# david-zwicker/video-analysis

Measured on AMD Instinct MI355X. Metric: frames/sec (bg-sub+blur+thresh+CCL) 1080p uint8, higher is better.
Workload: dtype u8; 1 GPU; cfg3_1080p_full_chain: 1920x1080 uint8, batch 256/GPU, running-mean bg-sub (f64 state) + sigma=5 Gaussian (q8.8) + threshold 20 + 5x5 dilate/erode + 4-connected labelling + object counts; inputs resident in HBM; engine=bg=1 gauss=mfma-i8(ksize=31) thresh=20 morph=2 ccl=4, video=one clip per rank, overlap=off, world_size=1, backend=single process

## Files before the change

video-analysis_amd/csrc/va_api.hip:

```cpp
#include <dlfcn.h>
#include <stdarg.h>
#include <stdlib.h>

#include <mutex>
#include <vector>
#include <new>

#include "va_common.h"

namespace va {

static thread_local char g_err[512] = "";

void set_error(const char *fmt, ...)
{
    va_list ap;
    va_start(ap, fmt);
    vsnprintf(g_err, sizeof(g_err), fmt, ap);
    va_end(ap);
}
const char *get_error() { return g_err; }

struct ScratchBlock {
    void *ptr;
    size_t bytes;
    hipStream_t st;
};
static std::mutex g_scratch_mu;
static std::vector<ScratchBlock> g_scratch_free;
static size_t g_scratch_cached = 0;
constexpr size_t kScratchCacheCap = 6ull << 30;

static void scratch_release_all_locked()
{
    for (const ScratchBlock &b : g_scratch_free)
        (void)hipFree(b.ptr);
    g_scratch_free.clear();
    g_scratch_cached = 0;
}

struct ScratchLease {
// ... 394 lines not shown
        return rc;
    return launch_gaussian(g, src, dst, nullptr, -1, 0, scratch.ptr, n, as_stream(stream), nullptr);
}

int va_gaussian_u8(const uint8_t *src, uint8_t *dst, int n, int h, int w, int c, double sigma,
                   void *stream)
{
    return va_gaussian_u8_rule(src, dst, n, h, w, c, sigma, VA_TAPS_CV4, stream);
}

int va_gaussian_u8_rule(const uint8_t *src, uint8_t *dst, int n, int h, int w, int c, double sigma,
                        int tap_rule, void *stream)
{
    return gaussian_call("va_gaussian_u8", VA_U8, src, dst, n, h, w, c, sigma, tap_rule, GaussFamily::None,
                         stream);
}

int va_gaussian_u8_generic(const uint8_t *src, uint8_t *dst, int n, int h, int w, int c,
                           double sigma, void *stream)
{
    return gaussian_call("va_gaussian_u8_generic", VA_U8, src, dst, n, h, w, c, sigma, VA_TAPS_CV4,
                         GaussFamily::U8Generic, stream);
}

int va_gaussian_u8_valu(const uint8_t *src, uint8_t *dst, int n, int h, int w, int c, double sigma,
                        void *stream)
{
    return gaussian_call("va_gaussian_u8_valu", VA_U8, src, dst, n, h, w, c, sigma, VA_TAPS_CV4,
                         GaussFamily::U8Dot, stream);
}

int va_test_hook_labelling(int path, int lds_runs)
{
    VA_REQUIRE(path >= 0 && path <= 4 && lds_runs >= 0, "va_test_hook_labelling: bad arguments");
    ccl_test_hook(path, lds_runs);
    return VA_OK;
}

static int g_gauss_u8_valu = 0;
int va_test_hook_gaussian_u8(int force_valu)
{
    g_gauss_u8_valu = force_valu != 0;
    return VA_OK;
}

int va_test_hook_gaussian_f32(int generic_columns)
{
    gauss_f32_test_hook(generic_columns);
    return VA_OK;
}

int va_gaussian_f32(const float *src, float *dst, int n, int h, int w, int c, double sigma,
                    void *stream)
{
    return gaussian_call("va_gaussian_f32", VA_F32, src, dst, n, h, w, c, sigma, VA_TAPS_CV4, GaussFamily::None,
                         stream);
}

int va_bg_update(int mode, int dtype, const void *frames, void *diff_out, void *state,
                 int64_t n_seen, double rate, int n, size_t px, void *stream)
{
    VA_ENTER();
    double *recip = nullptr;
    ScratchLease scratch;
    if (mode == VA_BG_MEAN && dtype == VA_U8 && n > 0) {
        int rc = scratch.acquire(bg_scratch_bytes(n), as_stream(stream));
        if (rc)
// ... 882 lines not shown
    uint32_t *const *bits = p->bits[slot];

    bool have_bits = false;
    if (c.sigma > 0) {
        if (p->gauss.byte_mask() && masks && mask_out && !filtered_out && c.morph_count == 0 && !want_ccl &&
            reinterpret_cast<uintptr_t>(mask_out) % 4 == 0) {
            return launch_gaussian(p->gauss, cur, mask_out, nullptr, c.thresh, c.maxval, p->gscratch, n, st, prof);
        }
        uint32_t *gbits = masks && p->gauss.single_pass() ? bits[0] : nullptr;
        void *dst = filtered_out ? filtered_out : p->blur;
        rc = launch_gaussian(p->gauss, cur, dst, gbits, c.thresh, 0, p->gscratch, n, st, prof);
        if (rc)
            return rc;
        have_bits = gbits != nullptr;
        cur = dst;
    } else if (filtered_out) {
        VA_HIP(hipMemcpyAsync(filtered_out, cur, (size_t)n * p->px * esz, hipMemcpyDeviceToDevice,
                              st));
    }
    if (!masks)
        return VA_OK;

    int b = 0;
    if (!have_bits) {
        rc = launch_pack_bits((const uint8_t *)cur, bits[0], n, c.height, c.width, c.thresh, st);
        if (rc)
            return rc;
        VA_MARK("threshold_pack");
    }
    int32_t *labels = nullptr;
    if (want_ccl) {
        labels = labels_out ? labels_out : p->labels_scratch;
    }
    if (c.morph_count > 0 && morph_fused_supported(c.width, p->se, c.morph_count)) {
        rc = launch_morph_fused(bits[b], bits[b ^ 1], n, c.height, c.width, c.morph_op, p->se,
                                c.morph_count, st);
        if (rc)
            return rc;
        b ^= 1;
        VA_MARK("morph_fused");
    } else {
        for (int i = 0; i < c.morph_count; i++) {
            rc = launch_morph_bits(bits[b], bits[b ^ 1], n, c.height, c.width, c.morph_op[i],
                                   p->se[i], st);
            if (rc)
                return rc;
            b ^= 1;
            VA_MARK(c.morph_op[i] == VA_MORPH_DILATE ? "morph_dilate" : "morph_erode");
        }
    }
    if (mask_out) {
        rc = launch_unpack_bits(bits[b], mask_out, n, c.height, c.width, c.maxval, st);
        if (rc)
            return rc;
        VA_MARK("mask_unpack");
    }
    if (want_ccl) {
        const bool paint = labels_out != nullptr || stats_out != nullptr;
        int32_t *counts = counts_out ? counts_out : p->counts_scratch;
        const char *lo = (const char *)labels, *hi = lo + (size_t)n * p->frame_px * sizeof(int32_t);
        const char *slo = (const char *)stats_out,
                   *shi = slo + (stats_out ? (size_t)n * c.max_labels * VA_STATS_STRIDE * sizeof(int64_t) : 0);
        for (int s = 0; s < 2 && p->overlap; s++)
            if (p->paint_pending[s] &&
                ((lo < p->paint_hi[s] && p->paint_lo[s] < hi) || (slo < p->pstat_hi[s] && p->pstat_lo[s] < shi)))
                VA_HIP(hipStreamWaitEvent(st, p->ev_paint[s], 0));
        if (!defer_paint) {
            rc = launch_ccl(bits[b], labels, counts, n, c.height, c.width, c.connectivity, p->ccl_ws[0],
                            p->ccl_ws_bytes, stats_out, c.max_labels, st, prof, paint);
            if (rc)
                return rc;
        } else {
            CclPaintPlan plan;
            rc = launch_ccl_front(bits[b], labels, counts, n, c.height, c.width, c.connectivity, p->ccl_ws[slot],
                                  p->ccl_ws_bytes, stats_out, c.max_labels, st, prof, &plan);
            if (rc)
                return rc;
            VA_HIP(hipEventRecord(p->ev_front, st));
            VA_HIP(hipStreamWaitEvent(p->side, p->ev_front, 0));
            if (prof)
                prof->mark(nullptr, p->side);
            plan.persistent_grid = p->paint_grid;
            rc = launch_ccl_paint(plan, p->side, prof);
            if (rc)
                return rc;
            VA_HIP(hipEventRecord(p->ev_paint[slot], p->side));
            p->paint_pending[slot] = true;
            p->paint_lo[slot] = lo;
            p->paint_hi[slot] = hi;
            p->pstat_lo[slot] = slo;
            p->pstat_hi[slot] = shi;
            p->slot = slot ^ 1;
        }
    }
#undef VA_MARK
    return VA_OK;
}

int va_pipeline_profile(va_pipeline_t *p, int enable)
{
    VA_ENTER();
    VA_REQUIRE(p, "va_pipeline_profile: NULL pipeline");
    if (!p->prof) {
        p->prof = new (std::nothrow) StageProfiler();
        if (!p->prof) {
            set_error("va_pipeline_profile: out of host memory");
            return VA_ERR_NOMEM;
        }
// ... 154 lines not shown
```

video-analysis_amd/csrc/va_ccl.hip:

```cpp
#include "va_common.h"

namespace va {

namespace {

constexpr int kBlock = 256;
constexpr int kRowsPerBlock = kBlock / kWave;
constexpr bool kNtStores = true;

__device__ __forceinline__ int ld_forest(const int32_t *p)
{
    return __hip_atomic_load(p, __ATOMIC_RELAXED, __HIP_MEMORY_SCOPE_WORKGROUP);
}
__device__ __forceinline__ void st_forest(int32_t *p, int v)
{
    __hip_atomic_store(p, v, __ATOMIC_RELAXED, __HIP_MEMORY_SCOPE_WORKGROUP);
}

__device__ int find_root(int32_t *L, int a)
{
    for (;;) {
        int p = ld_forest(L + a);
        if (p == a)
            return a;
        int gp = ld_forest(L + p);
        if (gp == p)
            return p;
        st_forest(L + a, gp);
        a = gp;
    }
}

__device__ int find_root_ro(const int32_t *L, int a)
// ... 547 lines not shown
        all += p;
    }
    if (threadIdx.x == 0)
        *total = all;
    __syncthreads();
    return before + incl - v;
}

__device__ __forceinline__ void scan_rows(int *rowbase, int h, int *s_part, int *total)
{
    const int per = (h + kFrameThreads - 1) / kFrameThreads;
    const int y0 = min(h, (int)threadIdx.x * per), y1 = min(h, y0 + per);
    int sum = 0;
    for (int y = y0; y < y1; y++)
        sum += rowbase[y];
    int run = block_exclusive_scan(sum, s_part, total);
    for (int y = y0; y < y1; y++) {
        const int n = rowbase[y];
        rowbase[y] = run;
        run += n;
    }
    __syncthreads();
}

#ifdef VA_CCL_STAMPS
__device__ long long g_ccl_stamps[16];
__device__ int g_ccl_xcc[2][16];
#define CCL_ACC(v, t0) do { long long t1_ = __builtin_amdgcn_s_memtime(); v += t1_ - t0; t0 = t1_; } while (0)
#define CCL_STAMP(i) do { if (blockIdx.x == 0 && threadIdx.x == 0) g_ccl_stamps[i] = __builtin_amdgcn_s_memtime(); } while (0)
#else
#define CCL_STAMP(i) do { } while (0)
#define CCL_ACC(v, t0) do { } while (0)
#endif
template <bool CONN8, int NCH, int RPW>
__global__ void __launch_bounds__(kFrameThreads)
ccl_frame_kernel(const uint32_t *__restrict__ bits, int32_t *__restrict__ labels,
                 int32_t *__restrict__ counts, int h, int w, int w32, FrameLayout lay, int direct,
                 int32_t *__restrict__ table, int table_stride, int32_t *__restrict__ rowbase_g,
                 int32_t *__restrict__ mode)
{
    __shared__ __attribute__((aligned(16))) int s_mem[kFrameLdsWords];
    __shared__ int s_part[kFrameWaves];
    __shared__ int s_total;

    const int f = blockIdx.x, tid = threadIdx.x, wv = tid >> 6, lane = tid & (kWave - 1);
#ifdef VA_CCL_STAMPS
    if (tid == 0 && f < 16)
        g_ccl_xcc[0][f] = __builtin_amdgcn_s_getreg((3 << 11) | 20) & 15;
#endif
    const uint32_t *fbits = bits + (size_t)f * h * w32;
    int32_t *L = labels + (size_t)f * h * w;
    int *stage = s_mem + wv * lay.stage_words + kStagePad;
    const int rs = lay.row_stride;
    const bool spans_direct = NCH == 1 && direct;
    if (!spans_direct)
        for (int i = lane; i < lay.stage_words; i += kWave)
            stage[i - kStagePad] = 0;
    int *queue = s_mem + lay.queue_off + wv * 2 * kQueue;
    int *rowbase = s_mem + lay.rowbase_off;
    int *parent = s_mem + lay.parent_off;
    constexpr int kRowsPerIter = kFrameWaves * RPW;
    const int sweeps = (h + kRowsPerIter - 1) / kRowsPerIter;

    typedef int v4i __attribute__((ext_vector_type(4)));
    struct RowRegs {
        v4i v[RPW + 1];
    };
    const int nld = (w32 + kWave - 1) / kWave;
    auto issue_rows = [&](int y0, RowRegs &rr) {
        const int c0 = min(lane, w32 - 1), c1 = min(lane + kWave, w32 - 1);
        const int c2 = min(lane + 2 * kWave, w32 - 1), c3 = min(lane + 3 * kWave, w32 - 1);
#pragma unroll
        for (int j = 0; j <= RPW; j++) {
            const uint32_t *src = fbits + (size_t)min(max(y0 - 1 + j, 0), h - 1) * w32;
            rr.v[j].x = (int)src[c0];
            if (nld > 1)
                rr.v[j].y = (int)src[c1];
            if (nld > 2) {
                rr.v[j].z = (int)src[c2];
                rr.v[j].w = (int)src[c3];
            }
        }
    };
// ... 976 lines not shown
        if (n++ == 0) {
            x = px;
            y = py;
        }
    }
};

__global__ void longest_contour_start_kernel(const uint32_t *__restrict__ bits,
                                             const unsigned long long *__restrict__ best_idx, int h, int w,
                                             int w32, int32_t *__restrict__ p1)
{
    const int f = blockIdx.x;
    if (threadIdx.x != 0)
        return;
    const unsigned long long key = best_idx[f];
    FirstEmit e;
    if (key != 0) {
        const int idx = (int)key - 1;
        BitImage im{bits + (size_t)f * h * w32, h, w, w32};
        trace_outer_border(im, idx % w, idx / w, e);
    }
    p1[2 * f] = e.x;
    p1[2 * f + 1] = e.y;
}

inline bool aligned(const void *p, size_t a) { return (reinterpret_cast<uintptr_t>(p) % a) == 0; }

}

static int g_ccl_path = 0;
static int g_ccl_lds_runs = 0;
static int g_ccl_sparse = 0;
static int g_ccl_no_direct = 0;
void ccl_test_hook(int path, int lds_runs)
{
    g_ccl_sparse = path == 3;
    g_ccl_no_direct = path == 4;
    g_ccl_path = path == 4 ? 2 : path == 3 ? 0 : path;
    g_ccl_lds_runs = lds_runs;
}

static int frame_rows_per_wave(int h, int w32)
{
    if ((long long)h * w32 > kMaxFrameWords || w32 > 128)
        return 0;
    for (int rpw = 8; rpw >= 4; rpw >>= 1)
        if (span_chunks(w32, rpw) <= 2 &&
            frame_layout(h, w32, rpw).lds_runs >= (rpw == 8 ? kWantLdsRuns : kMinLdsRuns))
            return rpw;
    return span_chunks(w32, 8) <= 2 && frame_layout(h, w32, 8).lds_runs >= kMinLdsRuns ? 8 : 0;
}

bool ccl_frame_kernel_used(int n, int h, int w)
{
    if (g_ccl_path == 1)
        return false;
    const int rpw = frame_rows_per_wave(h, words_per_row(w));
    if (rpw == 0)
        return false;
    if (g_ccl_path != 2) {
        const double wf = (double)h * words_per_row(w) / 64800.0, fill = (double)min(n, 256) / 256.0;
        const double t_frame = wf * (rpw == 8 ? 0.04 + 0.066 * fill : 0.075) + 0.01;
        const double t_chip = 0.277 * wf * n / 256.0 + 0.03;
        if (t_frame >= t_chip)
            return false;
    }
    return true;
}

static inline size_t up256(size_t v) { return (v + 255) & ~(size_t)255; }
size_t ccl_rows_workspace_bytes(int n, int h)
{
    return 2 * up256((size_t)n * h * sizeof(int32_t)) + up256((size_t)n * kFrameLdsWords * sizeof(int32_t)) +
           up256((size_t)n * sizeof(int32_t));
}

size_t ccl_workspace_bytes(int n, int h, int w)
{
    size_t bits = (size_t)n * h * words_per_row(w) * sizeof(uint32_t);
    auto up = [](size_t v) { return (v + 255) & ~(size_t)255; };
    return up(bits) + ccl_rows_workspace_bytes(n, h);
}

int launch_ccl_front(const uint32_t *bits, int32_t *labels, int32_t *counts, int n, int h, int w,
                     int connectivity, void *workspace, size_t ws_bytes, int64_t *stats, int max_labels,
                     hipStream_t st, StageProfiler *prof, CclPaintPlan *plan)
{
    const bool paint = plan != nullptr;
    if (plan)
        plan->n = 0;
#define VA_MARK(nm)      \
    do {                 \
        if (prof)        \
            prof->mark(nm, st); \
    } while (0)
    VA_REQUIRE(connectivity == 4 || connectivity == 8, "label: connectivity must be 4 or 8 (got %d)",
               connectivity);
    VA_REQUIRE(bits && labels && workspace, "label: NULL argument");
    VA_REQUIRE((size_t)h * (size_t)w < kMaxFramePixels,
               "label: frames of %dx%d exceed the supported 2^29 pixels (32-bit buffer descriptors "
               "address h*w*4 bytes of labels)", w, h);
    if (n == 0 || h == 0 || w == 0)
        return VA_OK;
    const int w32 = words_per_row(w);
    const size_t total_rows = (size_t)n * h;
    auto up = [](size_t v) { return (v + 255) & ~(size_t)255; };
    VA_REQUIRE(ws_bytes >= ccl_rows_workspace_bytes(n, h), "label: workspace too small");
    int32_t *row_cnt = (int32_t *)workspace;
    int32_t *row_off = (int32_t *)((char *)workspace + up(total_rows * sizeof(int32_t)));
    int32_t *run_table = (int32_t *)((char *)workspace + 2 * up(total_rows * sizeof(int32_t)));
    int32_t *frame_mode = (int32_t *)((char *)run_table + up((size_t)n * kFrameLdsWords * sizeof(int32_t)));
    bool table_mode = false;
    int table_stride = 0;

    const dim3 sgrid_all((unsigned)cdiv(h, kSparseRowsPerBlock), (unsigned)min(n, 4096));
    FrameList all{nullptr, nullptr, n};
    auto chip_wide = [&](const dim3 &sgrid, const FrameList &fl, int nscan, bool init) -> int {
        if (init) {
            ccl_init_kernel<<<sgrid, kBlock, 0, st>>>(bits, labels, h, w, w32, fl);
            VA_LAUNCH_CHECK("ccl_init_kernel");
            VA_MARK("ccl_init");
        }
        if (connectivity == 8)
            ccl_link_kernel<true><<<sgrid, kBlock, 0, st>>>(bits, labels, h, w, w32, fl);
        else
            ccl_link_kernel<false><<<sgrid, kBlock, 0, st>>>(bits, labels, h, w, w32, fl);
        VA_LAUNCH_CHECK("ccl_link_kernel");
        VA_MARK("ccl_link");
        ccl_flatten_kernel<<<sgrid, kBlock, 0, st>>>(bits, labels, row_cnt, h, w, w32, fl);
        VA_LAUNCH_CHECK("ccl_flatten_kernel");
        VA_MARK("ccl_flatten");
        ccl_rowscan_kernel<<<nscan, kBlock, 0, st>>>(row_cnt, row_off, counts, h, fl);
        VA_LAUNCH_CHECK("ccl_rowscan_kernel");
        VA_MARK("ccl_rowscan");
        ccl_rank_kernel<<<sgrid, kBlock, 0, st>>>(bits, labels, row_off, h, w, w32, fl);
        VA_LAUNCH_CHECK("ccl_rank_kernel");
        VA_MARK("ccl_rank");
        return VA_OK;
    };
    if (ccl_frame_kernel_used(n, h, w)) {
        const int rpw = frame_rows_per_wave(h, w32);
        FrameLayout lay = frame_layout(h, w32, rpw);
        if (g_ccl_lds_runs > 0)
            lay.lds_runs = min(lay.lds_runs, g_ccl_lds_runs);
        const int nch = span_chunks(w32, rpw);
        const int direct = nch == 1 && (w32 % 4 == 0) && aligned(bits, 16) && !g_ccl_no_direct;
        table_mode = paint && !g_ccl_sparse;
        table_stride = lay.lds_runs;
#define VA_FRAME_LAUNCH(C8, NCH, RPW)                                                                       \
    ccl_frame_kernel<C8, NCH, RPW><<<n, kFrameThreads, 0, st>>>(bits, labels, counts, h, w, w32, lay, direct,  \
                                                                 table_mode ? run_table : nullptr, lay.lds_runs, \
                                                                 row_off, frame_mode)
#define VA_FRAME_CASE(NCH, RPW)                 \
    if (nch == NCH && rpw == RPW) {             \
        if (connectivity == 8)                  \
            VA_FRAME_LAUNCH(true, NCH, RPW);    \
        else                                    \
            VA_FRAME_LAUNCH(false, NCH, RPW);   \
    }
        VA_FRAME_CASE(1, 8) VA_FRAME_CASE(2, 8) VA_FRAME_CASE(1, 4) VA_FRAME_CASE(2, 4)
#undef VA_FRAME_CASE
#undef VA_FRAME_LAUNCH
        VA_LAUNCH_CHECK("ccl_frame_kernel");
        VA_MARK("ccl_frame");
    } else {
        int rc = chip_wide(sgrid_all, all, n, true);
        if (rc)
            return rc;
    }
    if (!paint)
        return VA_OK;
    plan->bits = bits;
    plan->labels = labels;
    plan->n = n;
    plan->h = h;
    plan->w = w;
    plan->stats = stats;
    plan->max_labels = max_labels;
    plan->run_table = table_mode ? run_table : nullptr;
    plan->table_stride = table_stride;
    plan->row_off = row_off;
    plan->frame_mode = frame_mode;
    plan->xcd_frames = table_mode ? cdiv(h, kRowsPerBlock) : 0;
    plan->persistent_grid = 0;
#undef VA_MARK
    return VA_OK;
}

int launch_ccl_paint(const CclPaintPlan &pl, hipStream_t st, StageProfiler *prof)
{
#define VA_MARK(nm)      \
// ... 9 lines not shown
    const int grid = cdiv((long long)total_rows, kRowsPerBlock);
    const int vblocks = pl.xcd_frames ? 8 * pl.xcd_frames * cdiv(n, 8) : grid;
    const int pgrid = pl.persistent_grid > 0 ? min(vblocks, pl.persistent_grid) : vblocks;
    const bool wide = w32 > kWave && w32 <= 2 * kWave && vec && (w & 3) == 0 && (h & (kRowsPerBlock - 1)) == 0;
#define VA_PAINT_LAUNCH(ST, WORDS, STATSP, ML)                                                                      \
    ccl_paint_kernel<ST, WORDS><<<pgrid, kBlock, 0, st>>>(pl.bits, pl.labels, h, w, w32, total_rows, STATSP, ML, vec, \
                                                        pl.run_table, pl.table_stride, pl.row_off, pl.frame_mode,    \
                                                        pl.xcd_frames, vblocks)
    if (pl.stats && pl.max_labels > 0) {
        size_t entries = (size_t)n * pl.max_labels;
        stats_init_kernel<<<cdiv((long long)entries * VA_STATS_STRIDE, kBlock), kBlock, 0, st>>>(
            pl.stats, entries, h, w);
        VA_LAUNCH_CHECK("stats_init_kernel");
        VA_MARK("stats_init");
        if (wide)
            VA_PAINT_LAUNCH(true, 2 * kWave, pl.stats, pl.max_labels);
        else
            VA_PAINT_LAUNCH(true, kWave, pl.stats, pl.max_labels);
    } else {
        if (wide)
            VA_PAINT_LAUNCH(false, 2 * kWave, nullptr, 0);
        else
            VA_PAINT_LAUNCH(false, kWave, nullptr, 0);
    }
#undef VA_PAINT_LAUNCH
    VA_LAUNCH_CHECK("ccl_paint_kernel");
    VA_MARK("ccl_paint");
#undef VA_MARK
    return VA_OK;
}

int launch_ccl(const uint32_t *bits, int32_t *labels, int32_t *counts, int n, int h, int w,
               int connectivity, void *workspace, size_t ws_bytes, int64_t *stats, int max_labels,
               hipStream_t st, StageProfiler *prof, bool paint)
{
    CclPaintPlan plan;
    int rc = launch_ccl_front(bits, labels, counts, n, h, w, connectivity, workspace, ws_bytes, stats, max_labels,
                              st, prof, paint ? &plan : nullptr);
    if (rc || !paint)
        return rc;
    return launch_ccl_paint(plan, st, prof);
}

int launch_stats_from_labels(const int32_t *labels, int n, int h, int w, int max_labels,
                             int64_t *stats, hipStream_t st)
{
    VA_REQUIRE(labels && stats && max_labels > 0, "moments: NULL argument / max_labels <= 0");
    if (n == 0 || h == 0 || w == 0)
        return VA_OK;
    size_t entries = (size_t)n * max_labels;
    stats_init_kernel<<<cdiv((long long)entries * VA_STATS_STRIDE, kBlock), kBlock, 0, st>>>(
        stats, entries, h, w);
    VA_LAUNCH_CHECK("stats_init_kernel");
    const int w32 = words_per_row(w);
    size_t total_words = (size_t)n * h * w32;
    stats_from_labels_kernel<<<cdiv((long long)total_words, kBlock), kBlock, 0, st>>>(
        labels, h, w, w32, total_words, stats, max_labels);
    VA_LAUNCH_CHECK("stats_from_labels_kernel");
    return VA_OK;
}

int launch_largest_region(const int32_t *labels, const int32_t *counts, const int64_t *stats,
                          int n, int h, int w, int max_labels, int32_t *largest,
                          int64_t *largest_area, uint8_t *mask_out, hipStream_t st)
{
    VA_REQUIRE(counts && stats && largest && max_labels > 0, "largest_region: NULL argument");
    if (n == 0)
        return VA_OK;
    largest_label_kernel<<<n, kBlock, 0, st>>>(counts, stats, max_labels, largest, largest_area);
    VA_LAUNCH_CHECK("largest_label_kernel");
    if (mask_out) {
// ... 86 lines not shown
```

video-analysis_amd/csrc/va_common.h:

```cpp
#pragma once
#include <hip/hip_runtime.h>
#include <stdint.h>
#include <stdio.h>
#include <string.h>

#include "../../include/videoanalysis_hip.h"

namespace va {

void set_error(const char *fmt, ...) __attribute__((format(printf, 1, 2)));
const char *get_error();

inline hipStream_t as_stream(void *s) { return reinterpret_cast<hipStream_t>(s); }

#define VA_HIP(call)                                                                        \
    do {                                                                                    \
        hipError_t _e = (call);                                                             \
        if (_e != hipSuccess) {                                                             \
            va::set_error("%s failed: %s (%s:%d)", #call, hipGetErrorString(_e), __FILE__,  \
                          __LINE__);                                                        \
            return _e == hipErrorOutOfMemory ? VA_ERR_NOMEM : VA_ERR_HIP;                   \
        }                                                                                   \
    } while (0)

// ... 133 lines not shown
int launch_pack_bits(const uint8_t *src, uint32_t *bits, int n, int h, int w, int thresh,
                     hipStream_t st);
int launch_unpack_bits(const uint32_t *bits, uint8_t *dst, int n, int h, int w, int maxval,
                       hipStream_t st);

struct RowSpans {
    int ksize;
    int anchor;
    int8_t lo[64];
    int8_t hi[64];
};
int make_row_spans(int shape, int ksize, RowSpans *out);
int launch_morph_u8(const uint8_t *src, uint8_t *dst, int n, int h, int w, int op,
                    const RowSpans &se, hipStream_t st, uint8_t *scratch = nullptr);
int launch_morph_bits(const uint32_t *src, uint32_t *dst, int n, int h, int w, int op,
                      const RowSpans &se, hipStream_t st);

int launch_detect_peaks(const uint8_t *src, uint8_t *dst, int n, int h, int w, int include_plateaus,
                        hipStream_t st);
int launch_detect_peaks_f32(const float *src, uint8_t *dst, int n, int h, int w, int include_plateaus,
                            hipStream_t st);
int launch_image_statistics_f32(const float *src, double *mean_out, double *var_out, int n, int h, int w,
                                const RowSpans &se, double prior, int exclude_center, hipStream_t st);
int launch_thinning_step(const uint8_t *img, uint8_t *eroded, uint8_t *skel, int n, int h, int w,
                         unsigned long long *nonzero, hipStream_t st);
size_t image_statistics_scratch_bytes(int n, int h, int w);
int launch_image_statistics(const uint8_t *src, double *mean_out, double *var_out, int n, int h,
                            int w, const RowSpans &se, double prior, int exclude_center,
                            void *scratch, hipStream_t st);

bool morph_fused_supported(int w, const RowSpans *se, int count);
int launch_morph_fused(const uint32_t *src, uint32_t *dst, int n, int h,
                       int w, const int *ops, const RowSpans *se, int count, hipStream_t st);

size_t ccl_workspace_bytes(int n, int h, int w);
bool ccl_frame_kernel_used(int n, int h, int w);
void ccl_test_hook(int path, int lds_runs);
size_t ccl_rows_workspace_bytes(int n, int h);
int launch_ccl(const uint32_t *bits, int32_t *labels, int32_t *counts, int n, int h, int w,
               int connectivity, void *workspace, size_t ws_bytes, int64_t *stats, int max_labels,
               hipStream_t st, StageProfiler *prof = nullptr,
               bool paint = true);
struct CclPaintPlan {
    const uint32_t *bits;
    int32_t *labels;
    int n, h, w;
    int64_t *stats;
    int max_labels;
    const int32_t *run_table, *row_off, *frame_mode;
    int table_stride, xcd_frames;
    int persistent_grid;
};
int launch_ccl_front(const uint32_t *bits, int32_t *labels, int32_t *counts, int n, int h, int w,
                     int connectivity, void *workspace, size_t ws_bytes, int64_t *stats, int max_labels,
                     hipStream_t st, StageProfiler *prof, CclPaintPlan *plan);
int launch_ccl_paint(const CclPaintPlan &plan, hipStream_t st, StageProfiler *prof = nullptr);
int launch_largest_contour(const uint32_t *bits, const int32_t *forest, int n, int h, int w,
                           unsigned long long *best_keys, int32_t *points, int max_points,
                           int32_t *npoints, double *area, hipStream_t st);
int edge_label_words(int h, int w);
int launch_invert_bits(const uint32_t *bits, uint32_t *inv, int n, int h, int w, hipStream_t st);
int launch_longest_external_start(const uint32_t *bits, const int32_t *forest, const int32_t *bg_labels,
                                  uint32_t *edge_bits, int n, int h, int w, unsigned long long *keys,
                                  int32_t *p1, hipStream_t st);
size_t geodesic_pairs_bytes(int n, int h, int w);
size_t geodesic_visited_bytes(int n, int h, int w);
bool geodesic_width_ok(int w);
int launch_distance_map(const uint8_t *fillable, int n, int h, int w, const int32_t *starts,
                        const int32_t *nstarts, int max_starts, const int32_t *ends, const int32_t *nends,
                        int max_ends, int32_t *out, unsigned long long *pairs, int32_t *sweeps, hipStream_t st);
int launch_distance_path(const int32_t *map, int n, int h, int w, const int32_t *end_points, int32_t *path,
                         int max_points, int32_t *npath, uint32_t *visited, hipStream_t st);
int launch_farthest_points(const uint8_t *mask, int n, int h, int w, const int32_t *p1_in, int32_t *p1_out,
                           int32_t *p2_out, int32_t *dist_out, int32_t *rounds_out, int32_t *path, int max_points,
                           int32_t *npath, unsigned long long *pairs, uint32_t *visited, bool default_start,
                           hipStream_t st);
int launch_normalize(const void *src, int src_dtype, void *dst, int dst_dtype, size_t count, double fmin,
                     double fmax, double alpha, double tmin, hipStream_t st);
int launch_prepare_u8(const uint8_t *src, uint8_t *dst, int n, int src_h, int src_w, int src_c, int left, int top,
                      int width, int height, int mono, int normalize, double fmin, double fmax, double alpha,
                      double tmin, hipStream_t st);
int launch_gaussian_noise(void *dst, int dtype, size_t count, double mean, double stdev, uint64_t seed,
                          uint64_t first_index, hipStream_t st);
size_t resize_scratch_bytes(int sh, int sw, int dh, int dw);
int launch_resize_u8(const uint8_t *src, uint8_t *dst, int n, int sh, int sw, int c, int dh, int dw, int mode,
                     void *scratch, hipStream_t st);
enum class ResizeStage { Both, Upload, Launch };
int launch_resize_f32(const float *src, float *dst, int n, int sh, int sw, int c, int dh, int dw, int mode,
// ... 36 lines not shown
```

video-analysis_amd/csrc/va_morph.hip:

```cpp
#include <math.h>

#include "va_common.h"

namespace va {

int make_row_spans(int shape, int ksize, RowSpans *out)
{
    VA_REQUIRE(ksize >= 1, "morphology: ksize must be >= 1 (got %d)", ksize);
    if (ksize > 63) {
        set_error("morphology: ksize %d > 63 is not supported", ksize);
        return VA_ERR_RANGE;
    }
    VA_REQUIRE(shape >= VA_SHAPE_RECT && shape <= VA_SHAPE_ELLIPSE, "morphology: bad shape %d",
               shape);
    out->ksize = ksize;
    out->anchor = ksize / 2;
    const int r = ksize / 2, c = ksize / 2;
    const double inv_r2 = r ? 1.0 / ((double)r * r) : 0.0;
    for (int i = 0; i < ksize; i++) {
        int j1 = 0, j2 = 0;
        if (shape == VA_SHAPE_RECT || (shape == VA_SHAPE_CROSS && i == r)) {
            j2 = ksize;
        } else if (shape == VA_SHAPE_CROSS) {
            j1 = c;
            j2 = j1 + 1;
        } else {
            int dy = i - r;
            if (abs(dy) <= r) {
                int dx = (int)lrint(c * sqrt((r * r - dy * dy) * inv_r2));
                j1 = c - dx > 0 ? c - dx : 0;
                j2 = c + dx + 1 < ksize ? c + dx + 1 : ksize;
            }
        }
        out->lo[i] = (int8_t)j1;
        out->hi[i] = (int8_t)j2;
// ... 259 lines not shown
                for (int wi = tx; wi < w32; wi += 64) {
                    uint32_t acc = border;
                    for (int i = i0; i < i1; i++) {
                        const uint32_t v = bufH[(y + i - a - rbase) * w32 + wi];
                        acc = dil ? (acc | v) : (acc & v);
                    }
                    if (wi == w32 - 1)
                        acc &= last_valid;
                    bufB[(y - rbase) * w32 + wi] = acc;
                }
            }
        } else {
            for (int y = lo + ty; y < hi; y += 4)
                for (int wi = tx; wi < w32; wi += 64)
                    bufB[(y - rbase) * w32 + wi] =
                        morph_word_lds(bufA, rbase, y, wi, h, w32, last_valid, se, dil);
        }
        __syncthreads();
        uint32_t *t = bufA;
        bufA = bufB;
        bufB = t;
    }

    const int yend = min(h, y0 + kBandRows);
    uint32_t *fdst = dst + (size_t)f * h * w32;
    for (int y = y0 + ty; y < yend; y += 4) {
        const uint32_t *row = bufA + (y - rbase) * w32;
        for (int wi = tx; wi < w32; wi += 64)
            fdst[(size_t)y * w32 + wi] = row[wi];
    }
}

constexpr int kStreamBand = 32;

template <int K>
__device__ __forceinline__ uint32_t hdilate(uint32_t l, uint32_t c, uint32_t r)
{
    uint32_t acc = c;
#pragma unroll
    for (int d = 1; d <= K / 2; d++) {
        acc |= __builtin_amdgcn_alignbit(r, c, d);
        acc |= __builtin_amdgcn_alignbit(c, l, 32 - d);
    }
    return acc;
}

constexpr int kStreamGroup = 8;

__device__ __forceinline__ uint32_t lane_left(uint32_t v)
{
    return __builtin_amdgcn_update_dpp(0u, v, 0x138 , 0xf, 0xf, true);
}
__device__ __forceinline__ uint32_t lane_right(uint32_t v)
{
    return __builtin_amdgcn_update_dpp(0u, v, 0x130 , 0xf, 0xf, true);
}

template <int K0, int K1>
__global__ void __launch_bounds__(kBlock)
morph_stream_kernel(const uint32_t *__restrict__ src, uint32_t *__restrict__ dst, int n, int h, int w,
                     int w32, int nbands, int nchunks, uint32_t flip_in, uint32_t flip_mid,
                     uint32_t flip_out)
{
    constexpr int A0 = K0 / 2, A1 = K1 / 2;
    constexpr int LO = K1 ? 2 : 1;
    constexpr int COLS = K1 ? 60 : 62;
    const int lane = threadIdx.x & 63;
    size_t item = (size_t)blockIdx.x * (kBlock / 64) + (threadIdx.x >> 6);
    const int chunk = (int)(item % nchunks);
    item /= nchunks;
    const int band = (int)(item % nbands);
    const size_t f = item / nbands;
    if (f >= (size_t)n)
        return;
    const int wi = chunk * COLS + lane - LO;
    const bool col_in = wi >= 0 && wi < w32;
    const bool col_store = col_in && lane >= LO && lane < LO + COLS;
    const int tail = w & 31;
    const uint32_t valid = !col_in ? 0u : (wi == w32 - 1 && tail ? (0xFFFFFFFFu >> (32 - tail)) : 0xFFFFFFFFu);
    const uint32_t *fsrc = src + f * (size_t)h * w32 + min(max(wi, 0), w32 - 1);
    uint32_t *fdst = dst + f * (size_t)h * w32;

    const int y0 = band * kStreamBand;
    if (y0 >= h)
        return;
    const int y_first = y0 - A0 - A1;
    const int y_last = min(h, y0 + kStreamBand) - 1 + A0 + A1;

    auto load_group = [&](int y, uint32_t (&g)[kStreamGroup]) {
#pragma unroll
        for (int k = 0; k < kStreamGroup; k++)
            g[k] = fsrc[(size_t)min(max(y + k, 0), h - 1) * w32];
#pragma unroll
        for (int k = 0; k < kStreamGroup; k++)
            g[k] = (y + k >= 0 && y + k < h) ? ((g[k] ^ flip_in) & valid) : 0u;
    };

    uint32_t win0[K0], win1[K1 ? K1 : 1];
#pragma unroll
    for (int k = 0; k < K0; k++)
        win0[k] = 0u;
#pragma unroll
    for (int k = 0; k < (K1 ? K1 : 1); k++)
        win1[k] = 0u;

    uint32_t cur[kStreamGroup], nxt[kStreamGroup];
    load_group(y_first, nxt);
    for (int yg = y_first; yg <= y_last; yg += kStreamGroup) {
#pragma unroll
        for (int k = 0; k < kStreamGroup; k++)
            cur[k] = nxt[k];
        if (yg + kStreamGroup <= y_last)
            load_group(yg + kStreamGroup, nxt);
#pragma unroll
        for (int k = 0; k < kStreamGroup; k++) {
            const int y = yg + k;
            if (y > y_last)
                break;
            const uint32_t c = cur[k], l = lane_left(c), r = lane_right(c);
#pragma unroll
            for (int j = 0; j + 1 < K0; j++)
                win0[j] = win0[j + 1];
            win0[K0 - 1] = hdilate<K0>(l, c, r);
            uint32_t v0 = 0u;
#pragma unroll
            for (int j = 0; j < K0; j++)
                v0 |= win0[j];
            const int ya = y - A0;
            uint32_t out;
            int yo;
            if constexpr (K1 == 0) {
                out = (v0 ^ flip_out) & valid;
                yo = ya;
            } else {
                const uint32_t t = (ya >= 0 && ya < h) ? ((v0 ^ flip_mid) & valid) : 0u;
                const uint32_t tl = lane_left(t), tr = lane_right(t);
#pragma unroll
                for (int j = 0; j + 1 < K1; j++)
                    win1[j] = win1[j + 1];
                win1[K1 ? K1 - 1 : 0] = hdilate<(K1 ? K1 : 1)>(tl, t, tr);
                uint32_t v1 = 0u;
#pragma unroll
                for (int j = 0; j < K1; j++)
                    v1 |= win1[j];
                out = (v1 ^ flip_out) & valid;
                yo = ya - A1;
            }
            if (col_store && yo >= y0 && yo < y0 + kStreamBand && yo < h)
                fdst[(size_t)yo * w32 + wi] = out;
        }
    }
}

template <bool DILATE>
__global__ void __launch_bounds__(kBlock)
morph_u8_kernel(const uint8_t *__restrict__ src, uint8_t *__restrict__ dst, int h, int w,
                size_t total, RowSpans se)
{
    size_t e = (size_t)blockIdx.x * kBlock + threadIdx.x;
    if (e >= total)
        return;
    const int x = (int)(e % w);
    const size_t rowi = e / w;
    const int y = (int)(rowi % h);
    const uint8_t *frame = src + (rowi - y) * (size_t)w;
    int best = DILATE ? 0 : 255;
    for (int i = 0; i < se.ksize; i++) {
        const int yy = y + i - se.anchor;
        if (yy < 0 || yy >= h)
            continue;
        int x0 = x + se.lo[i] - se.anchor, x1 = x + se.hi[i] - 1 - se.anchor;
        x0 = x0 < 0 ? 0 : x0;
        x1 = x1 >= w ? w - 1 : x1;
        const uint8_t *row = frame + (size_t)yy * w;
        for (int xx = x0; xx <= x1; xx++) {
            int v = row[xx];
            best = DILATE ? (v > best ? v : best) : (v < best ? v : best);
        }
    }
    dst[e] = (uint8_t)best;
}

inline bool aligned(const void *p, size_t a) { return (reinterpret_cast<uintptr_t>(p) % a) == 0; }

// ... 40 lines not shown
        return VA_OK;
    int grid = cdiv((long long)total, kBlock);
    if (op == VA_MORPH_DILATE)
        morph_bits_kernel<true><<<grid, kBlock, 0, st>>>(src, dst, h, w, w32, total, se);
    else
        morph_bits_kernel<false><<<grid, kBlock, 0, st>>>(src, dst, h, w, w32, total, se);
    VA_LAUNCH_CHECK("morph_bits_kernel");
    return VA_OK;
}

bool morph_fused_supported(int w, const RowSpans *se, int count)
{
    if (count < 1 || count > VA_MAX_MORPH_OPS)
        return false;
    int reach = 0;
    for (int k = 0; k < count; k++) {
        int a = se[k].anchor, b = se[k].ksize - 1 - se[k].anchor;
        reach += a > b ? a : b;
    }
    size_t lds = 3 * (size_t)(kBandRows + 2 * reach) * words_per_row(w) * sizeof(uint32_t);
    return reach <= 16 && lds <= 64 * 1024;
}

static bool is_rect_odd(const RowSpans &se, int kmax)
{
    if (!(se.ksize & 1) || se.ksize > kmax || se.ksize < 3)
        return false;
    for (int i = 0; i < se.ksize; i++)
        if (se.lo[i] != 0 || se.hi[i] != se.ksize)
            return false;
    return true;
}

template <int K0, int K1>
static int launch_stream(const uint32_t *src, uint32_t *dst, int n, int h, int w, const int *ops,
                         hipStream_t st)
{
    const int w32 = words_per_row(w);
    const int cols = K1 ? 60 : 62;
    const int nchunks = cdiv(w32, cols), nbands = cdiv(h, kStreamBand);
    const size_t items = (size_t)n * nbands * nchunks;
    const uint32_t e0 = ops[0] == VA_MORPH_ERODE ? 0xFFFFFFFFu : 0u;
    const uint32_t e1 = K1 ? (ops[1] == VA_MORPH_ERODE ? 0xFFFFFFFFu : 0u) : 0u;
    const uint32_t flip_in = e0, flip_mid = e0 ^ e1, flip_out = K1 ? e1 : e0;
    const int waves_per_block = kBlock / 64;
    const size_t blocks = (items + waves_per_block - 1) / waves_per_block;
    morph_stream_kernel<K0, K1><<<(unsigned)blocks, kBlock, 0, st>>>(
        src, dst, n, h, w, w32, nbands, nchunks, flip_in, flip_mid, flip_out);
    VA_LAUNCH_CHECK("morph_stream_kernel");
    return VA_OK;
}

int launch_morph_fused(const uint32_t *src, uint32_t *dst, int n, int h, int w, const int *ops,
                       const RowSpans *se, int count, hipStream_t st)
{
    VA_REQUIRE(morph_fused_supported(w, se, count), "fused morphology: unsupported sequence");
    if (n == 0 || h == 0 || w == 0)
        return VA_OK;
    if (count <= 2 && is_rect_odd(se[0], 7) && (count == 1 || is_rect_odd(se[1], 7))) {
        const int k0 = se[0].ksize, k1 = count == 2 ? se[1].ksize : 0;
#define VA_STREAM_CASE(A, B) \
    if (k0 == A && k1 == B)  \
        return launch_stream<A, B>(src, dst, n, h, w, ops, st);
        VA_STREAM_CASE(3, 0) VA_STREAM_CASE(5, 0) VA_STREAM_CASE(7, 0)
        VA_STREAM_CASE(3, 3) VA_STREAM_CASE(3, 5) VA_STREAM_CASE(3, 7)
        VA_STREAM_CASE(5, 3) VA_STREAM_CASE(5, 5) VA_STREAM_CASE(5, 7)
        VA_STREAM_CASE(7, 3) VA_STREAM_CASE(7, 5) VA_STREAM_CASE(7, 7)
#undef VA_STREAM_CASE
    }
    MorphSeq seq;
    memset(&seq, 0, sizeof(seq));
    seq.count = count;
    for (int k = 0; k < count; k++) {
        seq.op[k] = ops[k];
        seq.se[k] = se[k];
        int a = se[k].anchor, b = se[k].ksize - 1 - se[k].anchor;
        seq.reach_total += a > b ? a : b;
    }
    const int w32 = words_per_row(w);
    const int nbands = cdiv(h, kBandRows);
    const size_t lds = 3 * (size_t)(kBandRows + 2 * seq.reach_total) * w32 * sizeof(uint32_t);
    morph_fused_kernel<<<nbands * n, kBlock, lds, st>>>(src, dst, h, w, w32, nbands,
                                                       seq);
    VA_LAUNCH_CHECK("morph_fused_kernel");
    return VA_OK;
}

template <bool DILATE, bool VERT>
__global__ void __launch_bounds__(kBlock)
morph_u8_line_kernel(const uint8_t *__restrict__ src, uint8_t *__restrict__ dst, int h, int w, size_t total,
                     int ksize, int anchor)
{
    size_t e = (size_t)blockIdx.x * kBlock + threadIdx.x;
// ... 161 lines not shown
```

Measured before the change: 314,200 frames/s.

## Fold streaming morphological closing into the per-frame CCL kernel

```diff
diff --git a/video-analysis_amd/csrc/va_api.hip b/video-analysis_amd/csrc/va_api.hip
--- a/video-analysis_amd/csrc/va_api.hip
+++ b/video-analysis_amd/csrc/va_api.hip
@@ -7,6 +7,7 @@
 #include <new>
 
 #include "va_common.h"
+#include "va_morph_stream.h"
 
 namespace va {
 
@@ -467,7 +468,7 @@
 
 int va_test_hook_labelling(int path, int lds_runs)
 {
-    VA_REQUIRE(path >= 0 && path <= 4 && lds_runs >= 0, "va_test_hook_labelling: bad arguments");
+    VA_REQUIRE(path >= 0 && path <= 5 && lds_runs >= 0, "va_test_hook_labelling: bad arguments");
     ccl_test_hook(path, lds_runs);
     return VA_OK;
 }
@@ -1416,7 +1417,18 @@
     if (want_ccl) {
         labels = labels_out ? labels_out : p->labels_scratch;
     }
-    if (c.morph_count > 0 && morph_fused_supported(c.width, p->se, c.morph_count)) {
+    CclClosing closing = {};
+    const bool fold = want_ccl && !mask_out && c.morph_count > 0 &&
+                      morph_stream_case(p->se, c.morph_count, &closing.k0, &closing.k1) &&
+                      ccl_closing_folded(n, c.height, c.width);
+    if (fold) {
+        const MorphStreamFlips fl = morph_stream_flips(c.morph_op, closing.k1);
+        closing.raw = bits[b];
+        closing.flip_in = fl.in;
+        closing.flip_mid = fl.mid;
+        closing.flip_out = fl.out;
+        b ^= 1;
+    } else if (c.morph_count > 0 && morph_fused_supported(c.width, p->se, c.morph_count)) {
         rc = launch_morph_fused(bits[b], bits[b ^ 1], n, c.height, c.width, c.morph_op, p->se,
                                 c.morph_count, st);
         if (rc)
@@ -1451,13 +1463,14 @@
                 VA_HIP(hipStreamWaitEvent(st, p->ev_paint[s], 0));
         if (!defer_paint) {
             rc = launch_ccl(bits[b], labels, counts, n, c.height, c.width, c.connectivity, p->ccl_ws[0],
-                            p->ccl_ws_bytes, stats_out, c.max_labels, st, prof, paint);
+                            p->ccl_ws_bytes, stats_out, c.max_labels, st, prof, paint, fold ? &closing : nullptr);
             if (rc)
                 return rc;
         } else {
             CclPaintPlan plan;
             rc = launch_ccl_front(bits[b], labels, counts, n, c.height, c.width, c.connectivity, p->ccl_ws[slot],
-                                  p->ccl_ws_bytes, stats_out, c.max_labels, st, prof, &plan);
+                                  p->ccl_ws_bytes, stats_out, c.max_labels, st, prof, &plan,
+                                  fold ? &closing : nullptr);
             if (rc)
                 return rc;
             VA_HIP(hipEventRecord(p->ev_front, st));
diff --git a/video-analysis_amd/csrc/va_ccl.hip b/video-analysis_amd/csrc/va_ccl.hip
--- a/video-analysis_amd/csrc/va_ccl.hip
+++ b/video-analysis_amd/csrc/va_ccl.hip
@@ -1,4 +1,5 @@
 #include "va_common.h"
+#include "va_morph_stream.h"
 
 namespace va {
 
@@ -612,12 +613,32 @@
 #define CCL_STAMP(i) do { } while (0)
 #define CCL_ACC(v, t0) do { } while (0)
 #endif
-template <bool CONN8, int NCH, int RPW>
+struct FrameClosing {
+    const uint32_t *raw;
+    uint32_t *closed;
+    int k0, k1, nbands, band_rows, nchunks;
+    uint32_t flip_in, flip_mid, flip_out;
+};
+constexpr int kCloseGroup = 16;
+
+template <int K0, int K1>
+__device__ __forceinline__ void close_frame(const FrameClosing &cl, size_t frame_off, int h, int w, int w32, int wv)
+{
+    for (int item = wv; item < cl.nbands * cl.nchunks; item += kFrameWaves) {
+        const int band = item / cl.nchunks, chunk = item - band * cl.nchunks;
+        const int y0 = band * cl.band_rows;
+        if (y0 < h)
+            morph_stream_rows<K0, K1, kCloseGroup>(cl.raw + frame_off, cl.closed + frame_off, h, w, w32, y0,
+                                                   cl.band_rows, chunk, cl.flip_in, cl.flip_mid, cl.flip_out);
+    }
+}
+
+template <bool CONN8, int NCH, int RPW, bool CLOSE = false>
 __global__ void __launch_bounds__(kFrameThreads)
 ccl_frame_kernel(const uint32_t *__restrict__ bits, int32_t *__restrict__ labels,
                  int32_t *__restrict__ counts, int h, int w, int w32, FrameLayout lay, int direct,
                  int32_t *__restrict__ table, int table_stride, int32_t *__restrict__ rowbase_g,
-                 int32_t *__restrict__ mode)
+                 int32_t *__restrict__ mode, FrameClosing cl)
 {
     __shared__ __attribute__((aligned(16))) int s_mem[kFrameLdsWords];
     __shared__ int s_part[kFrameWaves];
@@ -628,7 +649,20 @@
     if (tid == 0 && f < 16)
         g_ccl_xcc[0][f] = __builtin_amdgcn_s_getreg((3 << 11) | 20) & 15;
 #endif
-    const uint32_t *fbits = bits + (size_t)f * h * w32;
+    const uint32_t *fbits = CLOSE ? cl.closed + (size_t)f * h * w32 : bits + (size_t)f * h * w32;
+    if constexpr (CLOSE) {
+        const size_t off = (size_t)f * h * w32;
+#define VA_CLOSE_CASE(A, B)                    \
+    if (cl.k0 == A && cl.k1 == B)              \
+        close_frame<A, B>(cl, off, h, w, w32, wv);
+        VA_CLOSE_CASE(3, 0) VA_CLOSE_CASE(5, 0) VA_CLOSE_CASE(7, 0)
+        VA_CLOSE_CASE(3, 3) VA_CLOSE_CASE(3, 5) VA_CLOSE_CASE(3, 7)
+        VA_CLOSE_CASE(5, 3) VA_CLOSE_CASE(5, 5) VA_CLOSE_CASE(5, 7)
+        VA_CLOSE_CASE(7, 3) VA_CLOSE_CASE(7, 5) VA_CLOSE_CASE(7, 7)
+#undef VA_CLOSE_CASE
+        asm volatile("s_waitcnt vmcnt(0)" ::: "memory");
+        __syncthreads();
+    }
     int32_t *L = labels + (size_t)f * h * w;
     int *stage = s_mem + wv * lay.stage_words + kStagePad;
     const int rs = lay.row_stride;
@@ -1671,11 +1705,13 @@
 static int g_ccl_lds_runs = 0;
 static int g_ccl_sparse = 0;
 static int g_ccl_no_direct = 0;
+static int g_ccl_no_fold = 0;
 void ccl_test_hook(int path, int lds_runs)
 {
     g_ccl_sparse = path == 3;
     g_ccl_no_direct = path == 4;
-    g_ccl_path = path == 4 ? 2 : path == 3 ? 0 : path;
+    g_ccl_no_fold = path == 5;
+    g_ccl_path = path == 4 ? 2 : (path == 3 || path == 5) ? 0 : path;
     g_ccl_lds_runs = lds_runs;
 }
 
@@ -1707,6 +1743,15 @@
     return true;
 }
 
+bool ccl_closing_folded(int n, int h, int w)
+{
+    if (g_ccl_no_fold || !ccl_frame_kernel_used(n, h, w))
+        return false;
+    if (g_ccl_path == 2)
+        return true;
+    return true;
+}
+
 static inline size_t up256(size_t v) { return (v + 255) & ~(size_t)255; }
 size_t ccl_rows_workspace_bytes(int n, int h)
 {
@@ -1723,7 +1768,7 @@
 
 int launch_ccl_front(const uint32_t *bits, int32_t *labels, int32_t *counts, int n, int h, int w,
                      int connectivity, void *workspace, size_t ws_bytes, int64_t *stats, int max_labels,
-                     hipStream_t st, StageProfiler *prof, CclPaintPlan *plan)
+                     hipStream_t st, StageProfiler *prof, CclPaintPlan *plan, const CclClosing *closing)
 {
     const bool paint = plan != nullptr;
     if (plan)
@@ -1736,6 +1781,8 @@
     VA_REQUIRE(connectivity == 4 || connectivity == 8, "label: connectivity must be 4 or 8 (got %d)",
                connectivity);
     VA_REQUIRE(bits && labels && workspace, "label: NULL argument");
+    VA_REQUIRE(!closing || (closing->raw && closing->raw != bits && ccl_closing_folded(n, h, w)),
+               "label: the closing form needs the per-frame kernel and two mask buffers");
     VA_REQUIRE((size_t)h * (size_t)w < kMaxFramePixels,
                "label: frames of %dx%d exceed the supported 2^29 pixels (32-bit buffer descriptors "
                "address h*w*4 bytes of labels)", w, h);
@@ -1786,16 +1833,33 @@
         const int direct = nch == 1 && (w32 % 4 == 0) && aligned(bits, 16) && !g_ccl_no_direct;
         table_mode = paint && !g_ccl_sparse;
         table_stride = lay.lds_runs;
-#define VA_FRAME_LAUNCH(C8, NCH, RPW)                                                                       \
-    ccl_frame_kernel<C8, NCH, RPW><<<n, kFrameThreads, 0, st>>>(bits, labels, counts, h, w, w32, lay, direct,  \
-                                                                 table_mode ? run_table : nullptr, lay.lds_runs, \
-                                                                 row_off, frame_mode)
-#define VA_FRAME_CASE(NCH, RPW)                 \
-    if (nch == NCH && rpw == RPW) {             \
-        if (connectivity == 8)                  \
-            VA_FRAME_LAUNCH(true, NCH, RPW);    \
-        else                                    \
-            VA_FRAME_LAUNCH(false, NCH, RPW);   \
+        FrameClosing cl = {};
+        if (closing) {
+            cl.raw = closing->raw;
+            cl.closed = const_cast<uint32_t *>(bits);
+            cl.k0 = closing->k0;
+            cl.k1 = closing->k1;
+            cl.nchunks = cdiv(w32, morph_stream_cols(cl.k1));
+            cl.nbands = max(1, kFrameWaves / cl.nchunks);
+            cl.band_rows = cdiv(h, cl.nbands);
+            cl.flip_in = closing->flip_in;
+            cl.flip_mid = closing->flip_mid;
+            cl.flip_out = closing->flip_out;
+        }
+#define VA_FRAME_LAUNCH(C8, NCH, RPW, CLOSE)                                                                      \
+    ccl_frame_kernel<C8, NCH, RPW, CLOSE><<<n, kFrameThreads, 0, st>>>(bits, labels, counts, h, w, w32, lay,       \
+                                                                        direct, table_mode ? run_table : nullptr, \
+                                                                        lay.lds_runs, row_off, frame_mode, cl)
+#define VA_FRAME_CASE(NCH, RPW)                        \
+    if (nch == NCH && rpw == RPW) {                    \
+        if (connectivity == 8 && closing)              \
+            VA_FRAME_LAUNCH(true, NCH, RPW, true);     \
+        else if (connectivity == 8)                    \
+            VA_FRAME_LAUNCH(true, NCH, RPW, false);    \
+        else if (closing)                              \
+            VA_FRAME_LAUNCH(false, NCH, RPW, true);    \
+        else                                           \
+            VA_FRAME_LAUNCH(false, NCH, RPW, false);   \
     }
         VA_FRAME_CASE(1, 8) VA_FRAME_CASE(2, 8) VA_FRAME_CASE(1, 4) VA_FRAME_CASE(2, 4)
 #undef VA_FRAME_CASE
@@ -1871,11 +1935,11 @@
 
 int launch_ccl(const uint32_t *bits, int32_t *labels, int32_t *counts, int n, int h, int w,
                int connectivity, void *workspace, size_t ws_bytes, int64_t *stats, int max_labels,
-               hipStream_t st, StageProfiler *prof, bool paint)
+               hipStream_t st, StageProfiler *prof, bool paint, const CclClosing *closing)
 {
     CclPaintPlan plan;
     int rc = launch_ccl_front(bits, labels, counts, n, h, w, connectivity, workspace, ws_bytes, stats, max_labels,
-                              st, prof, paint ? &plan : nullptr);
+                              st, prof, paint ? &plan : nullptr, closing);
     if (rc || !paint)
         return rc;
     return launch_ccl_paint(plan, st, prof);
diff --git a/video-analysis_amd/csrc/va_common.h b/video-analysis_amd/csrc/va_common.h
--- a/video-analysis_amd/csrc/va_common.h
+++ b/video-analysis_amd/csrc/va_common.h
@@ -189,15 +189,22 @@
 bool morph_fused_supported(int w, const RowSpans *se, int count);
 int launch_morph_fused(const uint32_t *src, uint32_t *dst, int n, int h,
                        int w, const int *ops, const RowSpans *se, int count, hipStream_t st);
+bool morph_stream_case(const RowSpans *se, int count, int *k0, int *k1);
 
 size_t ccl_workspace_bytes(int n, int h, int w);
 bool ccl_frame_kernel_used(int n, int h, int w);
 void ccl_test_hook(int path, int lds_runs);
 size_t ccl_rows_workspace_bytes(int n, int h);
+struct CclClosing {
+    const uint32_t *raw;
+    int k0, k1;
+    uint32_t flip_in, flip_mid, flip_out;
+};
+bool ccl_closing_folded(int n, int h, int w);
 int launch_ccl(const uint32_t *bits, int32_t *labels, int32_t *counts, int n, int h, int w,
                int connectivity, void *workspace, size_t ws_bytes, int64_t *stats, int max_labels,
                hipStream_t st, StageProfiler *prof = nullptr,
-               bool paint = true);
+               bool paint = true, const CclClosing *closing = nullptr);
 struct CclPaintPlan {
     const uint32_t *bits;
     int32_t *labels;
@@ -210,7 +217,7 @@
 };
 int launch_ccl_front(const uint32_t *bits, int32_t *labels, int32_t *counts, int n, int h, int w,
                      int connectivity, void *workspace, size_t ws_bytes, int64_t *stats, int max_labels,
-                     hipStream_t st, StageProfiler *prof, CclPaintPlan *plan);
+                     hipStream_t st, StageProfiler *prof, CclPaintPlan *plan, const CclClosing *closing = nullptr);
 int launch_ccl_paint(const CclPaintPlan &plan, hipStream_t st, StageProfiler *prof = nullptr);
 int launch_largest_contour(const uint32_t *bits, const int32_t *forest, int n, int h, int w,
                            unsigned long long *best_keys, int32_t *points, int max_points,
diff --git a/video-analysis_amd/csrc/va_morph.hip b/video-analysis_amd/csrc/va_morph.hip
--- a/video-analysis_amd/csrc/va_morph.hip
+++ b/video-analysis_amd/csrc/va_morph.hip
@@ -1,6 +1,7 @@
 #include <math.h>
 
 #include "va_common.h"
+#include "va_morph_stream.h"
 
 namespace va {
 
@@ -326,29 +327,7 @@
 }
 
 constexpr int kStreamBand = 32;
-
-template <int K>
-__device__ __forceinline__ uint32_t hdilate(uint32_t l, uint32_t c, uint32_t r)
-{
-    uint32_t acc = c;
-#pragma unroll
-    for (int d = 1; d <= K / 2; d++) {
-        acc |= __builtin_amdgcn_alignbit(r, c, d);
-        acc |= __builtin_amdgcn_alignbit(c, l, 32 - d);
-    }
-    return acc;
-}
-
 constexpr int kStreamGroup = 8;
-
-__device__ __forceinline__ uint32_t lane_left(uint32_t v)
-{
-    return __builtin_amdgcn_update_dpp(0u, v, 0x138 , 0xf, 0xf, true);
-}
-__device__ __forceinline__ uint32_t lane_right(uint32_t v)
-{
-    return __builtin_amdgcn_update_dpp(0u, v, 0x130 , 0xf, 0xf, true);
-}
 
 template <int K0, int K1>
 __global__ void __launch_bounds__(kBlock)
@@ -356,10 +335,6 @@
                      int w32, int nbands, int nchunks, uint32_t flip_in, uint32_t flip_mid,
                      uint32_t flip_out)
 {
-    constexpr int A0 = K0 / 2, A1 = K1 / 2;
-    constexpr int LO = K1 ? 2 : 1;
-    constexpr int COLS = K1 ? 60 : 62;
-    const int lane = threadIdx.x & 63;
     size_t item = (size_t)blockIdx.x * (kBlock / 64) + (threadIdx.x >> 6);
     const int chunk = (int)(item % nchunks);
     item /= nchunks;
@@ -367,83 +342,11 @@
     const size_t f = item / nbands;
     if (f >= (size_t)n)
         return;
-    const int wi = chunk * COLS + lane - LO;
-    const bool col_in = wi >= 0 && wi < w32;
-    const bool col_store = col_in && lane >= LO && lane < LO + COLS;
-    const int tail = w & 31;
-    const uint32_t valid = !col_in ? 0u : (wi == w32 - 1 && tail ? (0xFFFFFFFFu >> (32 - tail)) : 0xFFFFFFFFu);
-    const uint32_t *fsrc = src + f * (size_t)h * w32 + min(max(wi, 0), w32 - 1);
-    uint32_t *fdst = dst + f * (size_t)h * w32;
-
     const int y0 = band * kStreamBand;
     if (y0 >= h)
         return;
-    const int y_first = y0 - A0 - A1;
-    const int y_last = min(h, y0 + kStreamBand) - 1 + A0 + A1;
-
-    auto load_group = [&](int y, uint32_t (&g)[kStreamGroup]) {
-#pragma unroll
-        for (int k = 0; k < kStreamGroup; k++)
-            g[k] = fsrc[(size_t)min(max(y + k, 0), h - 1) * w32];
-#pragma unroll
-        for (int k = 0; k < kStreamGroup; k++)
-            g[k] = (y + k >= 0 && y + k < h) ? ((g[k] ^ flip_in) & valid) : 0u;
-    };
-
-    uint32_t win0[K0], win1[K1 ? K1 : 1];
-#pragma unroll
-    for (int k = 0; k < K0; k++)
-        win0[k] = 0u;
-#pragma unroll
-    for (int k = 0; k < (K1 ? K1 : 1); k++)
-        win1[k] = 0u;
-
-    uint32_t cur[kStreamGroup], nxt[kStreamGroup];
-    load_group(y_first, nxt);
-    for (int yg = y_first; yg <= y_last; yg += kStreamGroup) {
-#pragma unroll
-        for (int k = 0; k < kStreamGroup; k++)
-            cur[k] = nxt[k];
-        if (yg + kStreamGroup <= y_last)
-            load_group(yg + kStreamGroup, nxt);
-#pragma unroll
-        for (int k = 0; k < kStreamGroup; k++) {
-            const int y = yg + k;
-            if (y > y_last)
-                break;
-            const uint32_t c = cur[k], l = lane_left(c), r = lane_right(c);
-#pragma unroll
-            for (int j = 0; j + 1 < K0; j++)
-                win0[j] = win0[j + 1];
-            win0[K0 - 1] = hdilate<K0>(l, c, r);
-            uint32_t v0 = 0u;
-#pragma unroll
-            for (int j = 0; j < K0; j++)
-                v0 |= win0[j];
-            const int ya = y - A0;
-            uint32_t out;
-            int yo;
-            if constexpr (K1 == 0) {
-                out = (v0 ^ flip_out) & valid;
-                yo = ya;
-            } else {
-                const uint32_t t = (ya >= 0 && ya < h) ? ((v0 ^ flip_mid) & valid) : 0u;
-                const uint32_t tl = lane_left(t), tr = lane_right(t);
-#pragma unroll
-                for (int j = 0; j + 1 < K1; j++)
-                    win1[j] = win1[j + 1];
-                win1[K1 ? K1 - 1 : 0] = hdilate<(K1 ? K1 : 1)>(tl, t, tr);
-                uint32_t v1 = 0u;
-#pragma unroll
-                for (int j = 0; j < K1; j++)
-                    v1 |= win1[j];
-                out = (v1 ^ flip_out) & valid;
-                yo = ya - A1;
-            }
-            if (col_store && yo >= y0 && yo < y0 + kStreamBand && yo < h)
-                fdst[(size_t)yo * w32 + wi] = out;
-        }
-    }
+    morph_stream_rows<K0, K1, kStreamGroup>(src + f * (size_t)h * w32, dst + f * (size_t)h * w32, h, w, w32, y0,
+                                            kStreamBand, chunk, flip_in, flip_mid, flip_out);
 }
 
 template <bool DILATE>
@@ -550,17 +453,25 @@
     return true;
 }
 
+bool morph_stream_case(const RowSpans *se, int count, int *k0, int *k1)
+{
+    if (count < 1 || count > 2 || !is_rect_odd(se[0], 7) || (count == 2 && !is_rect_odd(se[1], 7)))
+        return false;
+    *k0 = se[0].ksize;
+    *k1 = count == 2 ? se[1].ksize : 0;
+    return true;
+}
+
 template <int K0, int K1>
 static int launch_stream(const uint32_t *src, uint32_t *dst, int n, int h, int w, const int *ops,
                          hipStream_t st)
 {
     const int w32 = words_per_row(w);
-    const int cols = K1 ? 60 : 62;
+    const int cols = morph_stream_cols(K1);
     const int nchunks = cdiv(w32, cols), nbands = cdiv(h, kStreamBand);
     const size_t items = (size_t)n * nbands * nchunks;
-    const uint32_t e0 = ops[0] == VA_MORPH_ERODE ? 0xFFFFFFFFu : 0u;
-    const uint32_t e1 = K1 ? (ops[1] == VA_MORPH_ERODE ? 0xFFFFFFFFu : 0u) : 0u;
-    const uint32_t flip_in = e0, flip_mid = e0 ^ e1, flip_out = K1 ? e1 : e0;
+    const MorphStreamFlips fl = morph_stream_flips(ops, K1);
+    const uint32_t flip_in = fl.in, flip_mid = fl.mid, flip_out = fl.out;
     const int waves_per_block = kBlock / 64;
     const size_t blocks = (items + waves_per_block - 1) / waves_per_block;
     morph_stream_kernel<K0, K1><<<(unsigned)blocks, kBlock, 0, st>>>(
@@ -575,8 +486,8 @@
     VA_REQUIRE(morph_fused_supported(w, se, count), "fused morphology: unsupported sequence");
     if (n == 0 || h == 0 || w == 0)
         return VA_OK;
-    if (count <= 2 && is_rect_odd(se[0], 7) && (count == 1 || is_rect_odd(se[1], 7))) {
-        const int k0 = se[0].ksize, k1 = count == 2 ? se[1].ksize : 0;
+    int k0, k1;
+    if (morph_stream_case(se, count, &k0, &k1)) {
 #define VA_STREAM_CASE(A, B) \
     if (k0 == A && k1 == B)  \
         return launch_stream<A, B>(src, dst, n, h, w, ops, st);
diff --git a/video-analysis_amd/csrc/va_morph_stream.h b/video-analysis_amd/csrc/va_morph_stream.h
--- /dev/null
+++ b/video-analysis_amd/csrc/va_morph_stream.h
@@ -0,0 +1,121 @@
+#pragma once
+#include "va_common.h"
+
+namespace va {
+
+constexpr int morph_stream_cols(int k1) { return k1 ? 60 : 62; }
+
+template <int K>
+__device__ __forceinline__ uint32_t hdilate(uint32_t l, uint32_t c, uint32_t r)
+{
+    uint32_t acc = c;
+#pragma unroll
+    for (int d = 1; d <= K / 2; d++) {
+        acc |= __builtin_amdgcn_alignbit(r, c, d);
+        acc |= __builtin_amdgcn_alignbit(c, l, 32 - d);
+    }
+    return acc;
+}
+
+__device__ __forceinline__ uint32_t lane_left(uint32_t v)
+{
+    return __builtin_amdgcn_update_dpp(0u, v, 0x138 , 0xf, 0xf, true);
+}
+__device__ __forceinline__ uint32_t lane_right(uint32_t v)
+{
+    return __builtin_amdgcn_update_dpp(0u, v, 0x130 , 0xf, 0xf, true);
+}
+
+template <int K0, int K1, int GROUP>
+__device__ __forceinline__ void morph_stream_rows(const uint32_t *fsrc_frame, uint32_t *fdst, int h, int w, int w32,
+                                                  int y0, int nrows, int chunk, uint32_t flip_in, uint32_t flip_mid,
+                                                  uint32_t flip_out)
+{
+    constexpr int A0 = K0 / 2, A1 = K1 / 2;
+    constexpr int LO = K1 ? 2 : 1;
+    constexpr int COLS = morph_stream_cols(K1);
+    const int lane = threadIdx.x & 63;
+    const int wi = chunk * COLS + lane - LO;
+    const bool col_in = wi >= 0 && wi < w32;
+    const bool col_store = col_in && lane >= LO && lane < LO + COLS;
+    const int tail = w & 31;
+    const uint32_t valid = !col_in ? 0u : (wi == w32 - 1 && tail ? (0xFFFFFFFFu >> (32 - tail)) : 0xFFFFFFFFu);
+    const uint32_t *fsrc = fsrc_frame + min(max(wi, 0), w32 - 1);
+
+    const int y_first = y0 - A0 - A1;
+    const int y_last = min(h, y0 + nrows) - 1 + A0 + A1;
+
+    auto load_group = [&](int y, uint32_t (&g)[GROUP]) {
+#pragma unroll
+        for (int k = 0; k < GROUP; k++)
+            g[k] = fsrc[(size_t)min(max(y + k, 0), h - 1) * w32];
+    };
+
+    uint32_t win0[K0], win1[K1 ? K1 : 1];
+#pragma unroll
+    for (int k = 0; k < K0; k++)
+        win0[k] = 0u;
+#pragma unroll
+    for (int k = 0; k < (K1 ? K1 : 1); k++)
+        win1[k] = 0u;
+
+    uint32_t cur[GROUP], nxt[GROUP];
+    load_group(y_first, nxt);
+    for (int yg = y_first; yg <= y_last; yg += GROUP) {
+#pragma unroll
+        for (int k = 0; k < GROUP; k++)
+            cur[k] = nxt[k];
+        if (yg + GROUP <= y_last)
+            load_group(yg + GROUP, nxt);
+#pragma unroll
+        for (int k = 0; k < GROUP; k++) {
+            const int y = yg + k;
+            if (y > y_last)
+                break;
+            const uint32_t c = (y >= 0 && y < h) ? ((cur[k] ^ flip_in) & valid) : 0u;
+            const uint32_t l = lane_left(c), r = lane_right(c);
+#pragma unroll
+            for (int j = 0; j + 1 < K0; j++)
+                win0[j] = win0[j + 1];
+            win0[K0 - 1] = hdilate<K0>(l, c, r);
+            uint32_t v0 = 0u;
+#pragma unroll
+            for (int j = 0; j < K0; j++)
+                v0 |= win0[j];
+            const int ya = y - A0;
+            uint32_t out;
+            int yo;
+            if constexpr (K1 == 0) {
+                out = (v0 ^ flip_out) & valid;
+                yo = ya;
+            } else {
+                const uint32_t t = (ya >= 0 && ya < h) ? ((v0 ^ flip_mid) & valid) : 0u;
+                const uint32_t tl = lane_left(t), tr = lane_right(t);
+#pragma unroll
+                for (int j = 0; j + 1 < K1; j++)
+                    win1[j] = win1[j + 1];
+                win1[K1 ? K1 - 1 : 0] = hdilate<(K1 ? K1 : 1)>(tl, t, tr);
+                uint32_t v1 = 0u;
+#pragma unroll
+                for (int j = 0; j < K1; j++)
+                    v1 |= win1[j];
+                out = (v1 ^ flip_out) & valid;
+                yo = ya - A1;
+            }
+            if (col_store && yo >= y0 && yo < y0 + nrows && yo < h)
+                fdst[(size_t)yo * w32 + wi] = out;
+        }
+    }
+}
+
+struct MorphStreamFlips {
+    uint32_t in, mid, out;
+};
+inline MorphStreamFlips morph_stream_flips(const int *ops, int k1)
+{
+    const uint32_t e0 = ops[0] == VA_MORPH_ERODE ? 0xFFFFFFFFu : 0u;
+    const uint32_t e1 = k1 ? (ops[1] == VA_MORPH_ERODE ? 0xFFFFFFFFu : 0u) : 0u;
+    return MorphStreamFlips{e0, e0 ^ e1, k1 ? e1 : e0};
+}
+
+}
```

New measurement: 314,200 frames/s (median of 6 runs). No clear change (+0.0%).
